# pliang279/factorized

Measured on AMD Instinct MI355X. Metric: training samples/sec (MOSI-shape, T=20, 3 modalities), higher is better.
Workload: dtype fp32; 1 GPU; MFM_KL_EF mosi canonical sizes, per-GPU B=32, T=20, D=325, train mode (fwd + joint loss + bwd + Adam), fp32 HIP; global_batch=32, seq_len=20, parallelism=dp1, params=477294, handover_failures=0, role_workgroups=True

## Files before the change

### factorized_amd/_lib.py

```python
import ctypes as C
import os

_HERE = os.path.dirname(os.path.abspath(__file__))
LIB_PATH = os.environ.get("MFM_LIB_PATH") or os.path.join(_HERE, "libmfm_hip.so")

MFM_KLEF_NPARAM = 78
MFM_LOSS_SLOTS = 8
MFM_MAX_SEQ = 6
ABI_VERSION = 5


class MfmError(RuntimeError):
    pass


class GemmDesc(C.Structure):
    _fields_ = [("a", C.c_void_p), ("b", C.c_void_p), ("c", C.c_void_p), ("c2", C.c_void_p),
                ("bias", C.c_void_p), ("bias2", C.c_void_p),
                ("a_sz", C.c_int64), ("a_sm", C.c_int64), ("a_sk", C.c_int64),
                ("b_sz", C.c_int64), ("b_sk", C.c_int64), ("b_sn", C.c_int64),
                ("c_sz", C.c_int64), ("ldc", C.c_int64), ("bias_sz", C.c_int64),
                ("m", C.c_int32), ("n", C.c_int32), ("k", C.c_int32), ("n_valid", C.c_int32),
                ("batch", C.c_int32), ("split_k", C.c_int32), ("accumulate", C.c_int32),
                ("alpha", C.c_float), ("a_bf16", C.c_int32), ("c_bf16", C.c_int32), ("reserved_", C.c_int32 * 2)]


class SeqDesc(C.Structure):
    _fields_ = [("gates", C.c_void_p), ("hs", C.c_void_p), ("cs", C.c_void_p),
                ("w_hh", C.c_void_p), ("w_ih", C.c_void_p), ("b_ih", C.c_void_p), ("b_hh", C.c_void_p),
                ("h_init", C.c_void_p), ("ld_init", C.c_int64),
                ("dh_ext", C.c_void_p), ("ld_dh", C.c_int64),
                ("d_h_init", C.c_void_p), ("ld_dinit", C.c_int64),
                ("h", C.c_int32), ("is_dec", C.c_int32), ("dc_ext", C.c_void_p), ("w_pack", C.c_void_p),
                ("store_bf16", C.c_int32), ("bf16_dot", C.c_int32), ("h_last", C.c_void_p)]


class MemDesc(C.Structure):
    _fields_ = [("a1", C.c_void_p), ("a2", C.c_void_p), ("chat", C.c_void_p),
                ("w1m", C.c_void_p), ("w2m", C.c_void_p), ("w1b", C.c_void_p), ("b1b", C.c_void_p),
                ("w2b", C.c_void_p), ("b2b", C.c_void_p),
                ("gam1", C.c_void_p), ("gam2", C.c_void_p), ("mems", C.c_void_p), ("mem_out", C.c_void_p),
                ("dmem_out", C.c_void_p), ("du1", C.c_void_p), ("du2", C.c_void_p), ("dchat", C.c_void_p),
                ("T", C.c_int32), ("B", C.c_int32), ("M", C.c_int32), ("H1", C.c_int32), ("H2", C.c_int32),
                ("train", C.c_int32), ("p1", C.c_float), ("p2", C.c_float), ("seed", C.c_uint64),
                ("seed_dev", C.c_void_p), ("ld_wm", C.c_int64), ("dchat_pre_tanh", C.c_int32), ("reserved_", C.c_int32)]


class AdamSpan(C.Structure):
    _fields_ = [("begin", C.c_int64), ("end", C.c_int64), ("step", C.c_int32), ("reserved", C.c_int32)]


MFM_ADAM_MAX_SPANS = 8


class SgdSpan(C.Structure):
    _fields_ = [("begin", C.c_int64), ("end", C.c_int64), ("lr", C.c_float), ("weight_decay", C.c_float),
                ("momentum", C.c_float), ("dampening", C.c_float), ("flags", C.c_int32), ("reserved", C.c_int32)]


MFM_SGD_MAX_SPANS = 112
MFM_SGD_NESTEROV, MFM_SGD_MAXIMIZE, MFM_SGD_FIRST = 1, 2, 4


class AdamExtSpan(C.Structure):
    _fields_ = [("begin", C.c_int64), ("end", C.c_int64), ("step", C.c_int32), ("flags", C.c_int32), ("lr", C.c_float),
                ("beta1", C.c_float), ("beta2", C.c_float), ("eps", C.c_float), ("weight_decay", C.c_float),
                ("reserved", C.c_int32)]


MFM_ADAMX_MAX_SPANS = 88
MFM_ADAMX_MAXIMIZE, MFM_ADAMX_AMSGRAD, MFM_ADAMX_DECOUPLED = 1, 2, 4


class ClipSpan(C.Structure):
    _fields_ = [("begin", C.c_int64), ("end", C.c_int64)]


MFM_CLIP_MAX_SPANS = 112
MFM_NORM_L2, MFM_NORM_INF, MFM_NORM_L1 = 0, 1, 2
MFM_AVG_SWA, MFM_AVG_EMA = 0, 1
MFM_KEEP_MIN, MFM_KEEP_MAX = 0, 1
MFM_KEEP_STATE_WORDS = 8
MFM_PLATEAU_MAX_GROUPS = 16
MFM_PLATEAU_MIN, MFM_PLATEAU_MAX = 0, 1
MFM_PLATEAU_REL, MFM_PLATEAU_ABS = 0, 1
MFM_PLATEAU_STATE_WORDS = 8


class PlateauGroups(C.Structure):
    _fields_ = [("lr", C.c_void_p * MFM_PLATEAU_MAX_GROUPS), ("min_lr", C.c_double * MFM_PLATEAU_MAX_GROUPS)]


class LossWeights(C.Structure):
    _fields_ = [("disc", C.c_float), ("gen_l", C.c_float), ("gen_a", C.c_float), ("gen_v", C.c_float), ("reg", C.c_float),
                ("write_disc_loss", C.c_int32)]


class PlanConfig(C.Structure):
    _fields_ = [("d_l", C.c_int32), ("d_a", C.c_int32), ("d_v", C.c_int32),
                ("zl", C.c_int32), ("za", C.c_int32), ("zv", C.c_int32), ("zy", C.c_int32),
                ("fl", C.c_int32), ("fa", C.c_int32), ("fv", C.c_int32), ("fy", C.c_int32),
                ("output_dim", C.c_int32), ("loss_kind", C.c_int32),
                ("T", C.c_int32), ("B", C.c_int32),
                ("lda_xl", C.c_float), ("lda_xa", C.c_float), ("lda_xv", C.c_float), ("lda_reg", C.c_float),
                ("drop_zy", C.c_float), ("drop_zl", C.c_float), ("drop_za", C.c_float),
                ("drop_zv", C.c_float), ("drop_y", C.c_float),
                ("reg_scale", C.c_float), ("precision", C.c_int32),
                ("variant", C.c_int32), ("hl", C.c_int32), ("ha", C.c_int32), ("hv", C.c_int32), ("mem_dim", C.c_int32),
                ("nn1", C.c_int32), ("nn2", C.c_int32), ("g1", C.c_int32), ("g2", C.c_int32),
                ("drop_nn1", C.c_float), ("drop_nn2", C.c_float), ("drop_g1", C.c_float), ("drop_g2", C.c_float)]


_SIGS = {
    "mfm_abi_version": (C.c_int, []),
    "mfm_last_error": (C.c_char_p, []),
    "mfm_device_cus": (C.c_int, []),
    "mfm_gemm_grouped_f32": (C.c_int, [C.POINTER(GemmDesc), C.c_int, C.c_void_p]),
    "mfm_gemm_grouped_bf16": (C.c_int, [C.POINTER(GemmDesc), C.c_int, C.c_void_p]),
    "mfm_lstm_pack_bytes": (C.c_int64, [C.c_int32, C.c_int32]),
    "mfm_lstm_pack_bf16": (C.c_int, [C.POINTER(SeqDesc), C.c_int, C.c_void_p]),
    "mfm_lstm_seq_fwd_bf16": (C.c_int, [C.POINTER(SeqDesc), C.c_int, C.c_int, C.c_int, C.c_void_p]),
    "mfm_lstm_seq_bwd_bf16": (C.c_int, [C.POINTER(SeqDesc), C.c_int, C.c_int, C.c_int, C.c_void_p]),
    "mfm_lstm_seq_fwd": (C.c_int, [C.POINTER(SeqDesc), C.c_int, C.c_int, C.c_int, C.c_void_p]),
    "mfm_lstm_seq_bwd": (C.c_int, [C.POINTER(SeqDesc), C.c_int, C.c_int, C.c_int, C.c_void_p]),
    "mfm_dw_bf16_lstm": (C.c_int, [C.c_void_p, C.c_int32, C.c_int32, C.c_void_p, C.c_int32, C.c_int32, C.c_void_p, C.c_int32,
                                   C.c_void_p, C.c_void_p, C.c_void_p, C.c_void_p, C.c_void_p, C.c_void_p]),
    "mfm_dw_f32_lstm": (C.c_int, [C.c_void_p, C.c_int32, C.c_int32, C.c_void_p, C.c_int32, C.c_int32, C.c_int32, C.c_void_p, C.c_int32,
                                  C.c_void_p, C.c_void_p, C.c_void_p, C.c_void_p, C.c_void_p, C.c_void_p]),
    "mfm_mmd_fwd_bwd": (C.c_int, [C.c_void_p, C.c_void_p, C.c_int32, C.c_int32, C.c_void_p, C.c_void_p, C.c_void_p]),
    "mfm_mfn_mem_fwd": (C.c_int, [C.POINTER(MemDesc), C.c_void_p]),
    "mfm_mfn_mem_bwd": (C.c_int, [C.POINTER(MemDesc), C.c_void_p]),
    "mfm_mse_fwd_bwd": (C.c_int, [C.c_void_p, C.c_void_p, C.c_int64, C.c_int64, C.c_int32, C.c_float,
                                  C.c_float, C.c_void_p, C.c_void_p, C.c_void_p]),
    "mfm_adam_flat": (C.c_int, [C.c_void_p, C.c_void_p, C.c_void_p, C.c_void_p, C.c_int64, C.c_int32,
                                C.c_float, C.c_float, C.c_float, C.c_float, C.c_float, C.c_void_p]),
    "mfm_adam_flat_spans": (C.c_int, [C.c_void_p, C.c_void_p, C.c_void_p, C.c_void_p, C.POINTER(AdamSpan), C.c_int32,
                                      C.c_float, C.c_float, C.c_float, C.c_float, C.c_float, C.c_void_p]),
    "mfm_adam_flat_guarded": (C.c_int, [C.c_void_p, C.c_void_p, C.c_void_p, C.c_void_p, C.c_int64, C.c_int32,
                                        C.c_float, C.c_float, C.c_float, C.c_float, C.c_float, C.c_void_p, C.c_void_p]),
    "mfm_adam_flat_dev": (C.c_int, [C.c_void_p, C.c_void_p, C.c_void_p, C.c_void_p, C.c_int64, C.c_void_p, C.c_void_p,
                                    C.c_float, C.c_float, C.c_float, C.c_float, C.c_void_p, C.c_void_p]),
    "mfm_adam_flat_spans_guarded": (C.c_int, [C.c_void_p, C.c_void_p, C.c_void_p, C.c_void_p, C.POINTER(AdamSpan), C.c_int32,
                                              C.c_float, C.c_float, C.c_float, C.c_float, C.c_float, C.c_void_p, C.c_void_p]),
    "mfm_sgd_flat_spans": (C.c_int, [C.c_void_p, C.c_void_p, C.c_void_p, C.POINTER(SgdSpan), C.c_int32, C.c_float, C.c_void_p]),
    "mfm_sgd_flat_spans_guarded": (C.c_int, [C.c_void_p, C.c_void_p, C.c_void_p, C.POINTER(SgdSpan), C.c_int32, C.c_float,
                                             C.c_void_p, C.c_void_p]),
    "mfm_adam_ext_flat_spans": (C.c_int, [C.c_void_p, C.c_void_p, C.c_void_p, C.c_void_p, C.c_void_p, C.POINTER(AdamExtSpan),
                                          C.c_int32, C.c_float, C.c_void_p]),
    "mfm_adam_ext_flat_spans_guarded": (C.c_int, [C.c_void_p, C.c_void_p, C.c_void_p, C.c_void_p, C.c_void_p,
                                                  C.POINTER(AdamExtSpan), C.c_int32, C.c_float, C.c_void_p, C.c_void_p]),
    "mfm_clip_workspace_floats": (C.c_int64, []),
    "mfm_clip_grad_norm_flat_spans": (C.c_int, [C.c_void_p, C.POINTER(ClipSpan), C.c_int32, C.c_int32, C.c_float, C.c_void_p,
                                                C.c_void_p, C.c_void_p, C.c_void_p]),
    "mfm_clip_grad_value_flat_spans": (C.c_int, [C.c_void_p, C.POINTER(ClipSpan), C.c_int32, C.c_float, C.c_void_p, C.c_void_p]),
    "mfm_avg_flat": (C.c_int, [C.c_void_p, C.c_void_p, C.c_int64, C.c_int64, C.c_int32, C.c_float, C.c_void_p, C.c_void_p,
                               C.c_void_p]),
    "mfm_keep_best_flat": (C.c_int, [C.c_void_p, C.c_void_p, C.c_int64, C.c_int64, C.c_int32, C.c_void_p, C.c_float, C.c_void_p,
                                     C.c_void_p]),
    "mfm_plateau_step": (C.c_int, [C.c_void_p, C.c_void_p, C.c_double, C.POINTER(PlateauGroups), C.c_int32, C.c_int32, C.c_int32,
                                   C.c_double, C.c_double, C.c_double, C.c_int32, C.c_int32, C.c_int32, C.c_void_p]),
    "mfm_dataset_gather": (C.c_int, [C.c_void_p, C.c_void_p, C.c_void_p, C.c_void_p, C.c_void_p, C.c_int64, C.c_int32, C.c_int32,
                                     C.c_int32, C.c_int32, C.c_int64, C.c_void_p]),
    "mfm_p2p_create": (C.c_int, [C.c_int32, C.c_int32, C.c_int64, C.POINTER(C.c_void_p)]),
    "mfm_p2p_handle_bytes": (C.c_int, []),
    "mfm_p2p_export": (C.c_int, [C.c_void_p, C.c_void_p]),
    "mfm_p2p_connect": (C.c_int, [C.c_void_p, C.c_void_p]),
    "mfm_p2p_local_base": (C.c_void_p, [C.c_void_p]),
    "mfm_p2p_connect_bases": (C.c_int, [C.c_void_p, C.POINTER(C.c_void_p)]),
    "mfm_p2p_allreduce": (C.c_int, [C.c_void_p, C.c_void_p, C.c_int64, C.c_void_p]),
    "mfm_p2p_allreduce_adam": (C.c_int, [C.c_void_p, C.c_void_p, C.c_void_p, C.c_void_p, C.c_void_p, C.c_int64,
                                         C.c_int32, C.c_float, C.c_float, C.c_float, C.c_float, C.c_float,
                                         C.c_void_p]),
    "mfm_p2p_allreduce_adam_guarded": (C.c_int, [C.c_void_p, C.c_void_p, C.c_void_p, C.c_void_p, C.c_void_p, C.c_int64,
                                                 C.c_int32, C.c_float, C.c_float, C.c_float, C.c_float, C.c_float,
                                                 C.c_int64, C.c_void_p]),
    "mfm_p2p_status": (C.c_int, [C.c_void_p, C.POINTER(C.c_int32)]),
    "mfm_p2p_wait_stats": (C.c_int, [C.c_void_p, C.POINTER(C.c_int64), C.c_int32]),
    "mfm_p2p_destroy": (None, [C.c_void_p]),
    "mfm_plan_num_params": (C.c_int, [C.c_int32]),
    "mfm_plan_set_gauss": (C.c_int, [C.c_void_p, C.c_void_p]),
    "mfm_plan_create": (C.c_int, [C.POINTER(PlanConfig), C.POINTER(C.c_int64), C.c_int64,
                                  C.POINTER(C.c_void_p)]),
    "mfm_plan_destroy": (None, [C.c_void_p]),
    "mfm_plan_workspace_bytes": (C.c_int64, [C.c_void_p]),
    "mfm_plan_init_workspace": (C.c_int, [C.c_void_p, C.c_void_p, C.c_void_p]),
    "mfm_plan_forward": (C.c_int, [C.c_void_p, C.c_void_p, C.c_void_p, C.c_void_p, C.c_int, C.c_uint64,
                                   C.c_void_p, C.c_void_p, C.c_void_p, C.c_void_p, C.c_void_p,
                                   C.c_void_p, C.c_void_p]),
    "mfm_plan_backward": (C.c_int, [C.c_void_p, C.c_void_p, C.c_void_p, C.c_void_p, C.c_int, C.c_void_p,
                                    C.c_void_p, C.c_void_p]),
    "mfm_plan_backward_ext": (C.c_int, [C.c_void_p] * 11),
    "mfm_plan_forward_train": (C.c_int, [C.c_void_p, C.c_void_p, C.c_void_p, C.c_uint64, C.c_void_p, C.c_void_p, C.c_void_p]),
    "mfm_plan_backward_weighted": (C.c_int, [C.c_void_p, C.c_void_p, C.c_void_p, C.c_void_p, C.POINTER(LossWeights),
                                             C.c_void_p, C.c_void_p, C.c_void_p]),
    "mfm_plan_out_layout": (C.c_int, [C.c_void_p, C.POINTER(C.c_int64)]),
    "mfm_plan_host_status": (C.c_int, [C.c_void_p, C.POINTER(C.POINTER(C.c_uint32))]),
    "mfm_plan_grad_step": (C.c_int, [C.c_void_p, C.c_void_p, C.c_void_p, C.c_void_p, C.c_void_p, C.c_uint64,
                                     C.c_void_p, C.c_void_p, C.c_void_p]),
    "mfm_plan_train_step": (C.c_int, [C.c_void_p, C.c_void_p, C.c_void_p, C.c_void_p, C.c_void_p,
                                      C.c_void_p, C.c_void_p, C.c_uint64, C.c_int32, C.c_float,
                                      C.c_float, C.c_void_p, C.c_void_p, C.c_void_p]),
    "mfm_plan_train_step_staged": (C.c_int, [C.c_void_p, C.c_void_p, C.c_void_p, C.c_void_p, C.c_void_p,
                                             C.c_void_p, C.c_void_p, C.c_uint64, C.c_int32, C.POINTER(AdamSpan),
                                             C.c_int32, C.c_float, C.c_float, C.c_void_p, C.c_void_p, C.c_void_p]),
    "mfm_plan_set_option": (C.c_int, [C.c_void_p, C.c_char_p, C.c_int64]),
    "mfm_plan_set_option_str": (C.c_int, [C.c_void_p, C.c_char_p, C.c_char_p]),
    "mfm_plan_get_option": (C.c_int, [C.c_void_p, C.c_char_p, C.POINTER(C.c_int64)]),
    "mfm_plan_state_layout": (C.c_int, [C.c_void_p, C.POINTER(C.c_int64)]),
    "mfm_plan_clear_status": (C.c_int, [C.c_void_p, C.c_void_p, C.c_void_p]),
    "mfm_plan_latent_layout": (C.c_int, [C.c_void_p, C.POINTER(C.c_int64)]),
    "mfm_plan_seq_layout": (C.c_int, [C.c_void_p, C.c_int32, C.POINTER(C.c_int64)]),
    "mfm_plan_mfn_layout": (C.c_int, [C.c_void_p, C.POINTER(C.c_int64)]),
    "mfm_plan_flops_per_step": (C.c_double, [C.c_void_p]),
    "mfm_plan_bytes_per_step": (C.c_double, [C.c_void_p]),
    "mfm_plan_set_timing": (C.c_int, [C.c_void_p, C.c_int]),
    "mfm_plan_set_timing_every": (C.c_int, [C.c_void_p, C.c_int]),
    "mfm_plan_num_kernels": (C.c_int, []),
    "mfm_plan_kernel_name": (C.c_char_p, [C.c_int]),
    "mfm_plan_collect_timing": (C.c_int, [C.c_void_p, C.POINTER(C.c_double), C.POINTER(C.c_int64)]),
    "mfm_timing_bracket_overhead_ms": (C.c_int, [C.c_void_p, C.POINTER(C.c_double)]),
    "mfm_plan_kernel_flops": (C.c_double, [C.c_void_p, C.c_int]),
}

_lib = None


def lib():
    global _lib
    if _lib is None:
        if not os.path.exists(LIB_PATH):
            raise MfmError(
                "factorized_amd: %s is missing. Build the gfx950 HIP library first:\n"
                "    python -c 'import __graft_entry__ as g; g.build()'   (or factorized_amd/csrc/build.sh)\n"
                "There is no CPU fallback for this package." % LIB_PATH)
        import torch
        L = C.CDLL(LIB_PATH)
        for name, (res, args) in _SIGS.items():
            fn = getattr(L, name)
            fn.restype = res
            fn.argtypes = args
        if L.mfm_abi_version() != ABI_VERSION:
            raise MfmError("libmfm_hip.so ABI version %d, binding expects %d" % (L.mfm_abi_version(), ABI_VERSION))
        _lib = L
    return _lib


def check(rc, what=""):
    if rc != 0:
        msg = lib().mfm_last_error()
        raise MfmError("%s failed (%d): %s" % (what or "libmfm_hip call", rc,
                                               msg.decode() if msg else "?"))


def exported_names():
    return list(_SIGS)
```

### factorized_amd/csrc/dec_fc1.hip

```cpp
#include <hip/hip_runtime.h>
#include "internal.h"
#include "lstamp.h"

namespace mfm {

constexpr int FC1_THREADS = 512;
constexpr int FC1_WAVES = 8;
constexpr int FC1_ROWS = 16;
constexpr int FC1_MAXF = 8;
constexpr int FC1_KS2W = 4;
constexpr int FC1_LD = 16 * FC1_MAXF + 4;
constexpr int FC1_OOB = 0x7FFFFFF0;

__device__ __forceinline__ float rnd_bf16(float x, bool on) { return on ? (float)(__bf16)x : x; }

__global__ __launch_bounds__(FC1_THREADS) void dec_fc1_kernel(const DecFc1Launch L) {
  __shared__ __attribute__((aligned(16))) float Ht[FC1_ROWS * FC1_LD];
  __shared__ __attribute__((aligned(16))) float Dx[FC1_ROWS * FC1_LD];
  __shared__ __attribute__((aligned(16))) float Pt[(FC1_WAVES / 2) * FC1_ROWS * FC1_LD];
  __shared__ float red[FC1_WAVES];
  LSTAMP(2, 0);
  int m = 0;
#pragma unroll
  for (int i = 1; i < 3; ++i)
    if (i < L.n_items && (int)blockIdx.x >= L.it[i].tile_begin) m = i;
  const DecFc1Item& I = L.it[m];
  const int d = I.d, h = I.h, Hp = I.Hp;
  const int local = (int)blockIdx.x - I.tile_begin;
  const int cg = local % I.col_groups;
  const int row0 = (local / I.col_groups) * FC1_ROWS;
  const int NF1 = (d + 15) >> 4;
  const int f0 = cg * I.frags_per_group, nfw = min(I.frags_per_group, NF1 - f0);
  const int tid = threadIdx.x, lane = tid & 63, wave = tid >> 6;
  const int bi = lane & 15, q = lane >> 4;
  const int J = Hp >> 4;

  const int per_row = Hp >> 2;
  const int hr = tid / per_row, hk = (tid - hr * per_row) << 2;
  f32x4 hreg = f32x4{0.f, 0.f, 0.f, 0.f};
  if (hr < FC1_ROWS && row0 + hr < L.rows) hreg = *reinterpret_cast<const f32x4*>(I.hs + (int64_t)(row0 + hr) * Hp + hk);
  const __amdgpu_buffer_rsrc_t wres = __builtin_amdgcn_make_buffer_rsrc((void*)I.w, 0, d * h * 4, 0x00020000);
  const int n = (f0 + wave) * 16 + bi;
  const bool cok = (int)(wave < nfw) & (int)(n < d);
  f32x4 w1[FC1_MAXF];
#pragma unroll
  for (int j = 0; j < FC1_MAXF; ++j) {
    const bool ok = (int)cok & (int)(j < J);
    w1[j] = __builtin_bit_cast(f32x4, __builtin_amdgcn_raw_buffer_load_b128(wres, ok ? (n * h + 16 * j + 4 * q) * 4 : FC1_OOB, 0, 0));
  }
  const int KS = nfw * 4;
  const int per = (KS + FC1_WAVES - 1) / FC1_WAVES;
  const int ks0 = wave * per;
  float w2[FC1_KS2W][FC1_MAXF];
#pragma unroll
  for (int i = 0; i < FC1_KS2W; ++i) {
    const int k = f0 * 16 + 4 * (ks0 + i) + q;
#pragma unroll
    for (int f = 0; f < FC1_MAXF; ++f) {
      const int c = f * 16 + bi;
      const bool ok = (int)(L.with_bwd != 0) & (int)(i < per) & (int)(ks0 + i < KS) & (int)(k < d) & (int)(c < h);
      w2[i][f] = __builtin_bit_cast(float, __builtin_amdgcn_raw_buffer_load_b32(wres, ok ? (k * h + c) * 4 : FC1_OOB, 0, 0));
    }
  }
  float xv[4];
#pragma unroll
  for (int r = 0; r < 4; ++r) {
    const int row = row0 + 4 * q + r;
    xv[r] = (cok && row < L.rows) ? I.x[(int64_t)row * I.ldx + n] : 0.0f;
  }
  const float bv = cok ? I.bias[n] : 0.0f;
  const bool rb = L.bf16 != 0;
  if (rb) {
#pragma unroll
    for (int e = 0; e < 4; ++e) hreg[e] = rnd_bf16(hreg[e], true);
  }
  if (hr < FC1_ROWS) *reinterpret_cast<f32x4*>(Ht + hr * FC1_LD + hk) = hreg;
  lds_barrier();
  LSTAMP(2, 1);

  f32x4 acc1 = f32x4{0.f, 0.f, 0.f, 0.f};
  if (wave < nfw) {
#pragma unroll
    for (int j = 0; j < FC1_MAXF; ++j) {
      const f32x4 hv = *reinterpret_cast<const f32x4*>(Ht + bi * FC1_LD + 16 * min(j, J - 1) + 4 * q);
#pragma unroll
      for (int e = 0; e < 4; ++e) acc1 = mma16x16x4(hv[e], rnd_bf16(w1[j][e], rb), acc1);
    }
  }
  float lsum = 0.0f;
  if (wave < nfw) {
#pragma unroll
    for (int r = 0; r < 4; ++r) {
      const int row = 4 * q + r;
      float dx = 0.0f;
      if (cok && row0 + row < L.rows) {
        const float xh = acc1[r] + bv;
        const float diff = xh - xv[r];
        lsum = fmaf(diff, diff, lsum);
        dx = I.grad_scale * diff;
        const int64_t o = (int64_t)(row0 + row) * d + n;
        if (I.xhat) I.xhat[o] = xh;
        if (I.dxhat) I.dxhat[o] = dx;
      }
      Dx[row * FC1_LD + wave * 16 + bi] = rnd_bf16(dx, rb);
    }
  }
#pragma unroll
  for (int o = 32; o >= 1; o >>= 1) lsum += __shfl_xor(lsum, o, 64);
  if (lane == 0) red[wave] = lsum;
  lds_barrier();
  if (tid == 0 && I.loss) {
    float s = 0.0f;
#pragma unroll
    for (int w = 0; w < FC1_WAVES; ++w) s += red[w];
    atomicAdd(I.loss, s * I.inv_count);
  }
  LSTAMP(2, 2);
  if (!L.with_bwd) return;

  {
    f32x4 acc2[FC1_MAXF];
#pragma unroll
    for (int f = 0; f < FC1_MAXF; ++f) acc2[f] = f32x4{0.f, 0.f, 0.f, 0.f};
#pragma unroll
    for (int i = 0; i < FC1_KS2W; ++i) {
      const float a = Dx[bi * FC1_LD + 4 * min(ks0 + i, KS - 1) + q];
#pragma unroll
      for (int f = 0; f < FC1_MAXF; ++f) acc2[f] = mma16x16x4(a, rnd_bf16(w2[i][f], rb), acc2[f]);
    }
    float* P = Pt + (wave & 3) * FC1_ROWS * FC1_LD;
    if (wave >= 4) {
#pragma unroll
      for (int f = 0; f < FC1_MAXF; ++f)
#pragma unroll
        for (int r = 0; r < 4; ++r) P[(4 * q + r) * FC1_LD + f * 16 + bi] = acc2[f][r];
    }
    lds_barrier();
    if (wave < 4) {
#pragma unroll
      for (int f = 0; f < FC1_MAXF; ++f)
#pragma unroll
        for (int r = 0; r < 4; ++r) P[(4 * q + r) * FC1_LD + f * 16 + bi] += acc2[f][r];
    }
  }
  lds_barrier();
  if (hr < FC1_ROWS && row0 + hr < L.rows) {
    f32x4 s = *reinterpret_cast<const f32x4*>(Pt + hr * FC1_LD + hk);
#pragma unroll
    for (int w = 1; w < FC1_WAVES / 2; ++w) s += *reinterpret_cast<const f32x4*>(Pt + (w * FC1_ROWS + hr) * FC1_LD + hk);
    float* o = I.dhs + (int64_t)(row0 + hr) * Hp + hk;
    if (I.col_groups == 1) {
      *reinterpret_cast<f32x4*>(o) = s;
    } else {
#pragma unroll
      for (int e = 0; e < 4; ++e) atomicAdd(o + e, s[e]);
    }
  }
  LSTAMP_W(2, 15);
}

int dec_fc1_launch(DecFc1Launch& L, bool dhs_zeroed, hipStream_t stream) {
  MFM_REQUIRE(L.n_items >= 1 && L.n_items <= 3 && L.rows >= 1, "dec fc1: bad launch");
  int tiles = 0;
  const int row_tiles = (L.rows + FC1_ROWS - 1) / FC1_ROWS;
  for (int i = 0; i < L.n_items; ++i) {
    DecFc1Item& I = L.it[i];
    MFM_REQUIRE(I.hs && I.w && I.bias && I.x && I.d >= 1 && I.h >= 1 && I.Hp >= I.h && (I.Hp & 15) == 0, "dec fc1: item %d", i);
    MFM_REQUIRE(!L.with_bwd || I.dhs, "dec fc1: item %d: backward without a dH buffer", i);
    if (I.Hp > 16 * FC1_MAXF || (int64_t)I.d * I.h >= ((int64_t)1 << 28)) return MFM_ERR_UNSUPPORTED;
    const int NF1 = (I.d + 15) >> 4;
    if (NF1 > FC1_MAXF && !(dhs_zeroed || !L.with_bwd)) return MFM_ERR_UNSUPPORTED;
    I.frags_per_group = std::min(FC1_MAXF, NF1);
    I.col_groups = (NF1 + I.frags_per_group - 1) / I.frags_per_group;
    I.tile_begin = tiles;
    tiles += row_tiles * I.col_groups;
  }
  LSTAMP_BIND();
  MFM_LAUNCH_TIMED(dec_fc1_kernel, dim3(tiles), dim3(FC1_THREADS), 0, stream, L);
  MFM_LAUNCH_CHECK("dec_fc1_kernel");
  return MFM_OK;
}

}
```

### factorized_amd/csrc/lstamp.h

```cpp
#pragma once
#ifndef MFM_LAUNCH_STAMP
#define MFM_LAUNCH_STAMP 0
#endif

#if MFM_LAUNCH_STAMP
#include <hip/hip_runtime.h>

namespace mfm {
constexpr int LST_KERNELS = 6;
constexpr int LST_BLOCKS = 512;
constexpr int LST_POINTS = 32;
namespace {
__device__ unsigned long long* g_lstamp;
}
unsigned long long* lstamp_buffer();
static inline void lstamp_bind() {
  static bool done = false;
  if (done) return;
  unsigned long long* p = lstamp_buffer();
  (void)hipMemcpyToSymbol(HIP_SYMBOL(g_lstamp), &p, sizeof(p));
  done = true;
}
__device__ __forceinline__ void lstamp(int kid, int point, bool wait_loads = false) {
  if (threadIdx.x < 64) {
    if (wait_loads) asm volatile("s_waitcnt vmcnt(0) lgkmcnt(0)" ::: "memory");
    if (threadIdx.x == 0 && blockIdx.x < LST_BLOCKS && point < LST_POINTS)
      g_lstamp[((long)kid * LST_BLOCKS + blockIdx.x) * LST_POINTS + point] = wall_clock64();
  }
}
}
#define LSTAMP(kid, pt) ::mfm::lstamp(kid, pt)
#define LSTAMP_W(kid, pt) ::mfm::lstamp(kid, pt, true)
#define LSTAMP_BIND() ::mfm::lstamp_bind()
#else
#define LSTAMP(kid, pt) ((void)0)
#define LSTAMP_W(kid, pt) ((void)0)
#define LSTAMP_BIND() ((void)0)
#endif
```

### include/mfm_hip.h

```cpp
#ifndef MFM_HIP_H_
#define MFM_HIP_H_

#include <stddef.h>
#include <stdint.h>

#ifdef __cplusplus
extern "C" {
#endif

#define MFM_OK 0
#define MFM_ERR_ARG (-1)
#define MFM_ERR_HIP (-2)
#define MFM_ERR_UNSUPPORTED (-3)

#define MFM_ABI_VERSION 5

int mfm_abi_version(void);
const char* mfm_last_error(void);
int mfm_device_cus(void);

typedef struct MfmGemmDesc {
  const float* a; const float* b; float* c; float* c2;
  const float* bias; const float* bias2;
  int64_t a_sz, a_sm, a_sk;
  int64_t b_sz, b_sk, b_sn;
  int64_t c_sz, ldc, bias_sz;
  int32_t m, n, k, n_valid, batch, split_k, accumulate;
  float alpha;
  int32_t a_bf16, c_bf16;
  int32_t reserved_[2];
} MfmGemmDesc;

int mfm_gemm_grouped_f32(const MfmGemmDesc* descs , int count, void* stream);
int mfm_gemm_grouped_bf16(const MfmGemmDesc* descs , int count, void* stream);

#define MFM_MAX_SEQ 6
typedef struct MfmSeqDesc {
  float* gates; float* hs; float* cs;
  const float* w_hh; const float* w_ih; const float* b_ih; const float* b_hh;
  const float* h_init; int64_t ld_init;
  const float* dh_ext;
  int64_t ld_dh;
  float* d_h_init;
  int64_t ld_dinit;
  int32_t h, is_dec;
  const float* dc_ext;
  void* w_pack;
  int32_t store_bf16;
  int32_t bf16_dot;
  float* h_last;
} MfmSeqDesc;

int mfm_lstm_seq_fwd(const MfmSeqDesc* descs , int count, int T, int B, void* stream);

int64_t mfm_lstm_pack_bytes(int32_t h, int32_t is_dec);
int mfm_lstm_pack_bf16(const MfmSeqDesc* descs , int count, void* stream);
int mfm_lstm_seq_fwd_bf16(const MfmSeqDesc* descs , int count, int T, int B, void* stream);
int mfm_lstm_seq_bwd_bf16(const MfmSeqDesc* descs , int count, int T, int B, void* stream);

int mfm_lstm_seq_bwd(const MfmSeqDesc* descs , int count, int T, int B, void* stream);

int mfm_dw_bf16_lstm(const void* dA, int32_t rows, int32_t h, const void* xb, int32_t ldx, int32_t dx, const void* hs,
                     int32_t shift, float* dw_ih, float* dw_hh, float* dw_hh2, float* db_ih, float* db_hh, void* stream);
int mfm_dw_f32_lstm(const float* dA, int32_t rows, int32_t h, const float* x, int32_t ldx, int32_t xcol0, int32_t dx,
                    const float* hs, int32_t shift, float* dw_ih, float* dw_hh, float* dw_hh2, float* db_ih, float* db_hh,
                    void* stream);

int mfm_mse_fwd_bwd(const float* xhat, const float* x, int64_t ldx, int64_t rows, int32_t d,
                    float inv_count, float grad_scale, float* dxhat, float* loss_slot, void* stream);

typedef struct MfmMemDesc {
  float* a1; float* a2;
  const float* chat;
  const float* w1m; const float* w2m;
  const float* w1b; const float* b1b;
  const float* w2b; const float* b2b;
  float* gam1; float* gam2; float* mems;
  float* mem_out;
  const float* dmem_out;
  float* du1; float* du2; float* dchat;
  int32_t T, B, M, H1, H2, train;
  float p1, p2;
  uint64_t seed;
  const uint64_t* seed_dev;
  int64_t ld_wm;
  int32_t dchat_pre_tanh;
  int32_t reserved_;
} MfmMemDesc;

int mfm_mfn_mem_fwd(const MfmMemDesc* desc , void* stream);
int mfm_mfn_mem_bwd(const MfmMemDesc* desc , void* stream);

int mfm_mmd_fwd_bwd(const float* z, const float* gauss, int32_t B, int32_t dim, float* loss ,
                    float* dz , void* stream);

int mfm_adam_flat(float* p, const float* g, float* m, float* v, int64_t n, int32_t step, float lr,
                  float beta1, float beta2, float eps, float grad_scale, void* stream);

int mfm_adam_flat_guarded(float* p, const float* g, float* m, float* v, int64_t n, int32_t step, float lr,
                          float beta1, float beta2, float eps, float grad_scale, const float* guard, void* stream);

int mfm_adam_flat_dev(float* p, const float* g, float* m, float* v, int64_t n, int32_t* step_dev, const float* lr_dev,
                      float beta1, float beta2, float eps, float grad_scale, const float* guard, void* stream);

#define MFM_ADAM_MAX_SPANS 8
typedef struct MfmAdamSpan { int64_t begin, end; int32_t step; int32_t reserved; } MfmAdamSpan;
int mfm_adam_flat_spans(float* p, const float* g, float* m, float* v, const MfmAdamSpan* spans , int32_t nspans,
                        float lr, float beta1, float beta2, float eps, float grad_scale, void* stream);
int mfm_adam_flat_spans_guarded(float* p, const float* g, float* m, float* v, const MfmAdamSpan* spans , int32_t nspans,
                                float lr, float beta1, float beta2, float eps, float grad_scale, const float* guard, void* stream);

#define MFM_SGD_MAX_SPANS 112
#define MFM_SGD_NESTEROV 1
#define MFM_SGD_MAXIMIZE 2
#define MFM_SGD_FIRST 4
typedef struct MfmSgdSpan {
  int64_t begin, end;
  float lr, weight_decay, momentum, dampening;
  int32_t flags;
  int32_t reserved;
} MfmSgdSpan;
int mfm_sgd_flat_spans(float* p, const float* g, float* buf, const MfmSgdSpan* spans , int32_t nspans, float grad_scale,
                       void* stream);
int mfm_sgd_flat_spans_guarded(float* p, const float* g, float* buf, const MfmSgdSpan* spans , int32_t nspans,
                               float grad_scale, const float* guard, void* stream);

#define MFM_ADAMX_MAX_SPANS 88
#define MFM_ADAMX_MAXIMIZE 1
#define MFM_ADAMX_AMSGRAD 2
#define MFM_ADAMX_DECOUPLED 4
typedef struct MfmAdamExtSpan {
  int64_t begin, end;
  int32_t step;
  int32_t flags;
  float lr, beta1, beta2, eps, weight_decay;
  int32_t reserved;
} MfmAdamExtSpan;
int mfm_adam_ext_flat_spans(float* p, const float* g, float* m, float* v, float* vmax, const MfmAdamExtSpan* spans ,
                            int32_t nspans, float grad_scale, void* stream);
int mfm_adam_ext_flat_spans_guarded(float* p, const float* g, float* m, float* v, float* vmax,
                                    const MfmAdamExtSpan* spans , int32_t nspans, float grad_scale, const float* guard,
                                    void* stream);

#define MFM_CLIP_MAX_SPANS 112
#define MFM_NORM_L2 0
#define MFM_NORM_INF 1
#define MFM_NORM_L1 2
typedef struct MfmClipSpan {
  int64_t begin, end;
} MfmClipSpan;
int64_t mfm_clip_workspace_floats(void);
int mfm_clip_grad_norm_flat_spans(float* g, const MfmClipSpan* spans , int32_t nspans, int32_t norm_kind, float max_norm,
                                  float* ws, float* total_norm , const float* guard, void* stream);
int mfm_clip_grad_value_flat_spans(float* g, const MfmClipSpan* spans , int32_t nspans, float clip_value,
                                   const float* guard, void* stream);

#define MFM_AVG_SWA 0
#define MFM_AVG_EMA 1
int mfm_avg_flat(float* avg, const float* p, int64_t begin, int64_t end, int32_t kind, float w, int64_t* n_averaged ,
                 int32_t* ticket , void* stream);

#define MFM_KEEP_MIN 0
#define MFM_KEEP_MAX 1
typedef struct MfmKeepBestState {
  float best_value;
  int32_t calls;
  int32_t best_call;
  int32_t taken;
  int32_t ticket;
  int32_t reserved_[3];
} MfmKeepBestState;
int mfm_keep_best_flat(float* best, const float* p, int64_t begin, int64_t end, int32_t mode, const float* metric_dev ,
                       float metric, MfmKeepBestState* state , void* stream);

#define MFM_PLATEAU_MAX_GROUPS 16
#define MFM_PLATEAU_MIN 0
#define MFM_PLATEAU_MAX 1
#define MFM_PLATEAU_REL 0
#define MFM_PLATEAU_ABS 1
typedef struct MfmPlateauState {
  double best;
  int32_t num_bad_epochs;
  int32_t cooldown_counter;
  int32_t last_epoch;
  int32_t reduced;
  int32_t reductions;
  int32_t reserved_;
} MfmPlateauState;
typedef struct MfmPlateauGroups {
  float* lr[MFM_PLATEAU_MAX_GROUPS];
  double min_lr[MFM_PLATEAU_MAX_GROUPS];
} MfmPlateauGroups;
int mfm_plateau_step(MfmPlateauState* state , const float* metric_dev , double metric,
                     const MfmPlateauGroups* groups , int32_t n_groups, int32_t mode, int32_t threshold_mode, double factor,
                     double threshold, double eps, int32_t patience, int32_t cooldown, int32_t epoch ,
                     void* stream);

int mfm_dataset_gather(float* X, void* y, const float* X_pool, const void* y_pool, const int64_t* perm , int64_t N,
                       int32_t nb, int32_t T, int32_t B, int32_t D, int64_t ybytes, void* stream);

int mfm_p2p_create(int32_t nranks , int32_t rank, int64_t max_elems, void** handle);
int mfm_p2p_handle_bytes(void);
int mfm_p2p_export(void* handle, void* out );
int mfm_p2p_connect(void* handle, const void* all_handles );
void* mfm_p2p_local_base(void* handle);
int mfm_p2p_connect_bases(void* handle, const void* const* bases );
int mfm_p2p_allreduce(void* handle, float* buf , int64_t n , void* stream);
int mfm_p2p_allreduce_adam(void* handle, float* grads, float* p, float* m, float* v, int64_t n, int32_t step,
                           float lr, float beta1, float beta2, float eps, float grad_scale, void* stream);
int mfm_p2p_allreduce_adam_guarded(void* handle, float* grads, float* p, float* m, float* v, int64_t n, int32_t step,
                                   float lr, float beta1, float beta2, float eps, float grad_scale, int64_t guard_index,
                                   void* stream);
int mfm_p2p_status(void* handle, int32_t* timed_out );
int mfm_p2p_wait_stats(void* handle, int64_t* out , int32_t reset);
void mfm_p2p_destroy(void* handle);

#define MFM_KLEF_NPARAM 78
#define MFM_LOSS_SLOTS 8

typedef struct MfmPlanConfig {
  int32_t d_l, d_a, d_v;
  int32_t zl, za, zv, zy;
  int32_t fl, fa, fv, fy;
  int32_t output_dim;
  int32_t loss_kind;
  int32_t T, B;
  float lda_xl, lda_xa, lda_xv, lda_reg;
  float drop_zy, drop_zl, drop_za, drop_zv, drop_y;
  float reg_scale;
  int32_t precision;
  int32_t variant;
  int32_t hl, ha, hv;
  int32_t mem_dim;
  int32_t nn1, nn2, g1, g2;
  float drop_nn1, drop_nn2, drop_g1, drop_g2;
} MfmPlanConfig;

typedef struct MfmPlan MfmPlan;

int mfm_plan_num_params(int32_t variant);
int mfm_plan_create(const MfmPlanConfig* cfg, const int64_t* param_offsets ,
                    int64_t n_params_total, MfmPlan** out);
int mfm_plan_set_gauss(MfmPlan* plan, const float* gauss);
void mfm_plan_destroy(MfmPlan* plan);
int64_t mfm_plan_workspace_bytes(const MfmPlan* plan);

int mfm_plan_init_workspace(MfmPlan* plan, void* workspace, void* stream);

int mfm_plan_forward(MfmPlan* plan, const float* params, const float* x, const void* y, int train,
                     uint64_t seed, void* workspace, float* xhat_l, float* xhat_a, float* xhat_v,
                     float* y_hat, float* losses, void* stream);

int mfm_plan_backward(MfmPlan* plan, const float* params, const float* x, const void* y, int stage,
                      void* workspace, float* grads, void* stream);

int mfm_plan_backward_ext(MfmPlan* plan, const float* params, const float* x, const float* d_xhat_l,
                          const float* d_xhat_a, const float* d_xhat_v, const float* d_yhat,
                          const float* d_reg, void* workspace, float* grads, void* stream);

typedef struct MfmLossWeights { float disc, gen_l, gen_a, gen_v, reg; int32_t write_disc_loss; } MfmLossWeights;
int mfm_plan_forward_train(MfmPlan* plan, const float* params, const float* x, uint64_t seed, void* workspace,
                           float* grads_to_zero, void* stream);
int mfm_plan_backward_weighted(MfmPlan* plan, const float* params, const float* x, const void* y,
                               const MfmLossWeights* w , void* workspace, float* grads, void* stream);
int mfm_plan_out_layout(const MfmPlan* plan, int64_t* out );

int mfm_plan_grad_step(MfmPlan* plan, const float* params, float* grads, const float* x, const void* y,
                       uint64_t seed, void* workspace, float* losses, void* stream);

int mfm_plan_train_step(MfmPlan* plan, float* params, float* grads, float* adam_m, float* adam_v,
                        const float* x, const void* y, uint64_t seed, int32_t step, float lr,
                        float grad_scale, void* workspace, float* losses, void* stream);

int mfm_plan_train_step_staged(MfmPlan* plan, float* params, float* grads, float* adam_m, float* adam_v,
                               const float* x, const void* y, uint64_t seed, int32_t stage,
                               const MfmAdamSpan* spans , int32_t nspans, float lr, float grad_scale,
                               void* workspace, float* losses, void* stream);

int mfm_plan_set_option(MfmPlan* plan, const char* key, int64_t value);
int mfm_plan_set_option_str(MfmPlan* plan, const char* key, const char* value);
int mfm_plan_get_option(const MfmPlan* plan, const char* key, int64_t* value);

int mfm_plan_state_layout(const MfmPlan* plan, int64_t* out );
int mfm_plan_host_status(MfmPlan* plan, uint32_t** out );
int mfm_plan_clear_status(MfmPlan* plan, void* workspace, void* stream);

int mfm_plan_latent_layout(const MfmPlan* plan, int64_t* out );

int mfm_plan_mfn_layout(const MfmPlan* plan, int64_t* out );

int mfm_plan_seq_layout(const MfmPlan* plan, int32_t which, int64_t* out );

double mfm_plan_flops_per_step(const MfmPlan* plan);
double mfm_plan_bytes_per_step(const MfmPlan* plan);

int mfm_plan_set_timing(MfmPlan* plan, int mask);
int mfm_plan_set_timing_every(MfmPlan* plan, int every);
int mfm_plan_num_kernels(void);
const char* mfm_plan_kernel_name(int kid);
int mfm_plan_collect_timing(MfmPlan* plan, double* sum_ms, int64_t* count);
int mfm_timing_bracket_overhead_ms(void* stream, double* ms_out);
double mfm_plan_kernel_flops(const MfmPlan* plan, int kid);

#ifdef __cplusplus
}
#endif
#endif
```

Measured before the change: 225,000 samples/s.

## Reuse fc1 weight fragments via LDS transpose for backward dgrad in decoder kernel

The decoder fc1 kernel no longer issues a second set of scalar global loads for the backward weight tile. Instead it writes the already-loaded forward weight fragments into a dynamic LDS buffer, transposed, and each wave computes one output column block of dhs directly, which removes the cross-wave partial-sum reduction and its extra barriers. The forward accumulation is split into four independent accumulators to shorten the MFMA dependency chain, and the xhat/dxhat stores are deferred until after the backward MMA. It also adds a C entry point and a Python binding for the kernel, plus timing stamp hooks. In exchange it needs more dynamic LDS per block, which may reduce occupancy.

```diff
diff --git a/factorized_amd/_lib.py b/factorized_amd/_lib.py
--- a/factorized_amd/_lib.py
+++ b/factorized_amd/_lib.py
@@ -74,6 +74,13 @@
 
 class ClipSpan(C.Structure):
     _fields_ = [("begin", C.c_int64), ("end", C.c_int64)]
+
+
+class DecFc1Item(C.Structure):
+    _fields_ = [("hs", C.c_void_p), ("w", C.c_void_p), ("bias", C.c_void_p), ("x", C.c_void_p),
+                ("xhat", C.c_void_p), ("dxhat", C.c_void_p), ("dhs", C.c_void_p), ("loss", C.c_void_p),
+                ("ldx", C.c_int64), ("d", C.c_int32), ("h", C.c_int32), ("Hp", C.c_int32),
+                ("inv_count", C.c_float), ("grad_scale", C.c_float), ("pad_", C.c_int32)]
 
 
 MFM_CLIP_MAX_SPANS = 112
@@ -153,6 +160,7 @@
     "mfm_clip_grad_norm_flat_spans": (C.c_int, [C.c_void_p, C.POINTER(ClipSpan), C.c_int32, C.c_int32, C.c_float, C.c_void_p,
                                                 C.c_void_p, C.c_void_p, C.c_void_p]),
     "mfm_clip_grad_value_flat_spans": (C.c_int, [C.c_void_p, C.POINTER(ClipSpan), C.c_int32, C.c_float, C.c_void_p, C.c_void_p]),
+    "mfm_dec_fc1_f32": (C.c_int, [C.POINTER(DecFc1Item), C.c_int32, C.c_int32, C.c_int32, C.c_int32, C.c_int32, C.c_void_p]),
     "mfm_avg_flat": (C.c_int, [C.c_void_p, C.c_void_p, C.c_int64, C.c_int64, C.c_int32, C.c_float, C.c_void_p, C.c_void_p,
                                C.c_void_p]),
     "mfm_keep_best_flat": (C.c_int, [C.c_void_p, C.c_void_p, C.c_int64, C.c_int64, C.c_int32, C.c_void_p, C.c_float, C.c_void_p,
diff --git a/factorized_amd/csrc/dec_fc1.hip b/factorized_amd/csrc/dec_fc1.hip
--- a/factorized_amd/csrc/dec_fc1.hip
+++ b/factorized_amd/csrc/dec_fc1.hip
@@ -1,4 +1,5 @@
 #include <hip/hip_runtime.h>
+#include <atomic>
 #include "internal.h"
 #include "lstamp.h"
 
@@ -8,7 +9,6 @@
 constexpr int FC1_WAVES = 8;
 constexpr int FC1_ROWS = 16;
 constexpr int FC1_MAXF = 8;
-constexpr int FC1_KS2W = 4;
 constexpr int FC1_LD = 16 * FC1_MAXF + 4;
 constexpr int FC1_OOB = 0x7FFFFFF0;
 
@@ -17,8 +17,8 @@
 __global__ __launch_bounds__(FC1_THREADS) void dec_fc1_kernel(const DecFc1Launch L) {
   __shared__ __attribute__((aligned(16))) float Ht[FC1_ROWS * FC1_LD];
   __shared__ __attribute__((aligned(16))) float Dx[FC1_ROWS * FC1_LD];
-  __shared__ __attribute__((aligned(16))) float Pt[(FC1_WAVES / 2) * FC1_ROWS * FC1_LD];
   __shared__ float red[FC1_WAVES];
+  extern __shared__ __attribute__((aligned(16))) float Wt[];
   LSTAMP(2, 0);
   int m = 0;
 #pragma unroll
@@ -34,6 +34,7 @@
   const int tid = threadIdx.x, lane = tid & 63, wave = tid >> 6;
   const int bi = lane & 15, q = lane >> 4;
   const int J = Hp >> 4;
+  const bool bwd = L.with_bwd != 0;
 
   const int per_row = Hp >> 2;
   const int hr = tid / per_row, hk = (tid - hr * per_row) << 2;
@@ -48,20 +49,6 @@
     const bool ok = (int)cok & (int)(j < J);
     w1[j] = __builtin_bit_cast(f32x4, __builtin_amdgcn_raw_buffer_load_b128(wres, ok ? (n * h + 16 * j + 4 * q) * 4 : FC1_OOB, 0, 0));
   }
-  const int KS = nfw * 4;
-  const int per = (KS + FC1_WAVES - 1) / FC1_WAVES;
-  const int ks0 = wave * per;
-  float w2[FC1_KS2W][FC1_MAXF];
-#pragma unroll
-  for (int i = 0; i < FC1_KS2W; ++i) {
-    const int k = f0 * 16 + 4 * (ks0 + i) + q;
-#pragma unroll
-    for (int f = 0; f < FC1_MAXF; ++f) {
-      const int c = f * 16 + bi;
-      const bool ok = (int)(L.with_bwd != 0) & (int)(i < per) & (int)(ks0 + i < KS) & (int)(k < d) & (int)(c < h);
-      w2[i][f] = __builtin_bit_cast(float, __builtin_amdgcn_raw_buffer_load_b32(wres, ok ? (k * h + c) * 4 : FC1_OOB, 0, 0));
-    }
-  }
   float xv[4];
 #pragma unroll
   for (int r = 0; r < 4; ++r) {
@@ -77,85 +64,104 @@
   if (hr < FC1_ROWS) *reinterpret_cast<f32x4*>(Ht + hr * FC1_LD + hk) = hreg;
   lds_barrier();
   LSTAMP(2, 1);
-
-  f32x4 acc1 = f32x4{0.f, 0.f, 0.f, 0.f};
-  if (wave < nfw) {
-#pragma unroll
-    for (int j = 0; j < FC1_MAXF; ++j) {
-      const f32x4 hv = *reinterpret_cast<const f32x4*>(Ht + bi * FC1_LD + 16 * min(j, J - 1) + 4 * q);
-#pragma unroll
-      for (int e = 0; e < 4; ++e) acc1 = mma16x16x4(hv[e], rnd_bf16(w1[j][e], rb), acc1);
-    }
-  }
+  LSTAMP_V(2, 10, 5);
+
+  f32x4 acc1[4];
+#pragma unroll
+  for (int e = 0; e < 4; ++e) acc1[e] = f32x4{0.f, 0.f, 0.f, 0.f};
+  float xh[4] = {0.f, 0.f, 0.f, 0.f}, dxr[4] = {0.f, 0.f, 0.f, 0.f};
   float lsum = 0.0f;
   if (wave < nfw) {
 #pragma unroll
+    for (int j = 0; j < FC1_MAXF; ++j) {
+      if (j < J) {
+        const f32x4 hv = *reinterpret_cast<const f32x4*>(Ht + bi * FC1_LD + 16 * j + 4 * q);
+        f32x4 wv;
+#pragma unroll
+        for (int e = 0; e < 4; ++e) wv[e] = rnd_bf16(w1[j][e], rb);
+#pragma unroll
+        for (int e = 0; e < 4; ++e) acc1[e] = mma16x16x4(hv[e], wv[e], acc1[e]);
+        if (bwd) {
+#pragma unroll
+          for (int e = 0; e < 4; ++e) {
+            const int u = 16 * j + 4 * q + e;
+            Wt[u * FC1_LD + wave * 16 + bi] = u < h ? wv[e] : 0.0f;
+          }
+        }
+      }
+    }
+    LSTAMP_W(2, 11);
+    const f32x4 s1 = (acc1[0] + acc1[1]) + (acc1[2] + acc1[3]);
+#pragma unroll
     for (int r = 0; r < 4; ++r) {
       const int row = 4 * q + r;
-      float dx = 0.0f;
+      xh[r] = s1[r] + bv;
+      dxr[r] = 0.0f;
       if (cok && row0 + row < L.rows) {
-        const float xh = acc1[r] + bv;
-        const float diff = xh - xv[r];
+        const float diff = xh[r] - xv[r];
         lsum = fmaf(diff, diff, lsum);
-        dx = I.grad_scale * diff;
-        const int64_t o = (int64_t)(row0 + row) * d + n;
-        if (I.xhat) I.xhat[o] = xh;
-        if (I.dxhat) I.dxhat[o] = dx;
-      }
-      Dx[row * FC1_LD + wave * 16 + bi] = rnd_bf16(dx, rb);
+        dxr[r] = I.grad_scale * diff;
+      }
+      Dx[row * FC1_LD + wave * 16 + bi] = rnd_bf16(dxr[r], rb);
     }
   }
 #pragma unroll
   for (int o = 32; o >= 1; o >>= 1) lsum += __shfl_xor(lsum, o, 64);
   if (lane == 0) red[wave] = lsum;
+  LSTAMP(2, 12);
   lds_barrier();
-  if (tid == 0 && I.loss) {
+  LSTAMP(2, 2);
+
+  f32x4 acc2[4];
+#pragma unroll
+  for (int e = 0; e < 4; ++e) acc2[e] = f32x4{0.f, 0.f, 0.f, 0.f};
+  const bool w2on = (int)bwd & (int)(wave < J);
+  if (w2on) {
+    f32x4 av[FC1_MAXF], wv[FC1_MAXF];
+#pragma unroll
+    for (int j = 0; j < FC1_MAXF; ++j) {
+      if (j < nfw) {
+        av[j] = *reinterpret_cast<const f32x4*>(Dx + bi * FC1_LD + 16 * j + 4 * q);
+        wv[j] = *reinterpret_cast<const f32x4*>(Wt + (wave * 16 + bi) * FC1_LD + 16 * j + 4 * q);
+      }
+    }
+#pragma unroll
+    for (int j = 0; j < FC1_MAXF; ++j) {
+      if (j < nfw) {
+#pragma unroll
+        for (int e = 0; e < 4; ++e) acc2[e] = mma16x16x4(av[j][e], wv[j][e], acc2[e]);
+      }
+    }
+  }
+  if (cok) {
+#pragma unroll
+    for (int r = 0; r < 4; ++r) {
+      const int row = row0 + 4 * q + r;
+      if (row < L.rows) {
+        const int64_t o = (int64_t)row * d + n;
+        if (I.xhat) I.xhat[o] = xh[r];
+        if (I.dxhat) I.dxhat[o] = dxr[r];
+      }
+    }
+  }
+  if (tid == FC1_THREADS - 64 && I.loss) {
     float s = 0.0f;
 #pragma unroll
     for (int w = 0; w < FC1_WAVES; ++w) s += red[w];
     atomicAdd(I.loss, s * I.inv_count);
   }
-  LSTAMP(2, 2);
-  if (!L.with_bwd) return;
-
-  {
-    f32x4 acc2[FC1_MAXF];
-#pragma unroll
-    for (int f = 0; f < FC1_MAXF; ++f) acc2[f] = f32x4{0.f, 0.f, 0.f, 0.f};
-#pragma unroll
-    for (int i = 0; i < FC1_KS2W; ++i) {
-      const float a = Dx[bi * FC1_LD + 4 * min(ks0 + i, KS - 1) + q];
-#pragma unroll
-      for (int f = 0; f < FC1_MAXF; ++f) acc2[f] = mma16x16x4(a, rnd_bf16(w2[i][f], rb), acc2[f]);
-    }
-    float* P = Pt + (wave & 3) * FC1_ROWS * FC1_LD;
-    if (wave >= 4) {
-#pragma unroll
-      for (int f = 0; f < FC1_MAXF; ++f)
-#pragma unroll
-        for (int r = 0; r < 4; ++r) P[(4 * q + r) * FC1_LD + f * 16 + bi] = acc2[f][r];
-    }
-    lds_barrier();
-    if (wave < 4) {
-#pragma unroll
-      for (int f = 0; f < FC1_MAXF; ++f)
-#pragma unroll
-        for (int r = 0; r < 4; ++r) P[(4 * q + r) * FC1_LD + f * 16 + bi] += acc2[f][r];
-    }
-  }
-  lds_barrier();
-  if (hr < FC1_ROWS && row0 + hr < L.rows) {
-    f32x4 s = *reinterpret_cast<const f32x4*>(Pt + hr * FC1_LD + hk);
-#pragma unroll
-    for (int w = 1; w < FC1_WAVES / 2; ++w) s += *reinterpret_cast<const f32x4*>(Pt + (w * FC1_ROWS + hr) * FC1_LD + hk);
-    float* o = I.dhs + (int64_t)(row0 + hr) * Hp + hk;
-    if (I.col_groups == 1) {
-      *reinterpret_cast<f32x4*>(o) = s;
-    } else {
-#pragma unroll
-      for (int e = 0; e < 4; ++e) atomicAdd(o + e, s[e]);
-    }
-  }
+  if (w2on) {
+    const f32x4 s2 = (acc2[0] + acc2[1]) + (acc2[2] + acc2[3]);
+    float* o = I.dhs + (int64_t)(row0 + 4 * q) * Hp + wave * 16 + bi;
+#pragma unroll
+    for (int r = 0; r < 4; ++r) {
+      if (row0 + 4 * q + r < L.rows) {
+        if (I.col_groups == 1) o[r * Hp] = s2[r];
+        else atomicAdd(o + r * Hp, s2[r]);
+      }
+    }
+  }
+  LSTAMP(2, 13);
   LSTAMP_W(2, 15);
 }
 
@@ -175,10 +181,37 @@
     I.tile_begin = tiles;
     tiles += row_tiles * I.col_groups;
   }
+  int max_hp = 0;
+  for (int i = 0; i < L.n_items; ++i) max_hp = std::max(max_hp, L.it[i].Hp);
+  const size_t smem = L.with_bwd ? (size_t)max_hp * FC1_LD * sizeof(float) : 0;
+  static std::atomic<unsigned long long> lds_attr_set{0};
+  int dev = 0;
+  MFM_HIP_CHECK(hipGetDevice(&dev));
+  const unsigned long long dev_bit = 1ull << (dev & 63);
+  if (!(lds_attr_set.load(std::memory_order_acquire) & dev_bit)) {
+    MFM_HIP_CHECK(hipFuncSetAttribute((const void*)dec_fc1_kernel, hipFuncAttributeMaxDynamicSharedMemorySize, 16 * FC1_MAXF * FC1_LD * (int)sizeof(float)));
+    lds_attr_set.fetch_or(dev_bit, std::memory_order_release);
+  }
   LSTAMP_BIND();
-  MFM_LAUNCH_TIMED(dec_fc1_kernel, dim3(tiles), dim3(FC1_THREADS), 0, stream, L);
+  MFM_LAUNCH_TIMED(dec_fc1_kernel, dim3(tiles), dim3(FC1_THREADS), smem, stream, L);
   MFM_LAUNCH_CHECK("dec_fc1_kernel");
   return MFM_OK;
 }
 
 }
+
+extern "C" int mfm_dec_fc1_f32(const MfmDecFc1Item* items, int32_t count, int32_t rows, int32_t with_bwd, int32_t bf16_operands,
+                               int32_t dhs_zeroed, void* stream) {
+  MFM_REQUIRE(items && count >= 1 && count <= 3, "dec fc1: 1..3 items");
+  mfm::DecFc1Launch L;
+  memset(&L, 0, sizeof(L));
+  L.n_items = count; L.rows = rows; L.with_bwd = with_bwd ? 1 : 0; L.bf16 = bf16_operands ? 1 : 0;
+  for (int i = 0; i < count; ++i) {
+    mfm::DecFc1Item& I = L.it[i];
+    const MfmDecFc1Item& s = items[i];
+    I.hs = s.hs; I.w = s.w; I.bias = s.bias; I.x = s.x; I.ldx = s.ldx;
+    I.xhat = s.xhat; I.dxhat = s.dxhat; I.dhs = s.dhs; I.loss = s.loss;
+    I.d = s.d; I.h = s.h; I.Hp = s.Hp; I.inv_count = s.inv_count; I.grad_scale = s.grad_scale;
+  }
+  return mfm::dec_fc1_launch(L, dhs_zeroed != 0, (hipStream_t)stream);
+}
diff --git a/factorized_amd/csrc/lstamp.h b/factorized_amd/csrc/lstamp.h
--- a/factorized_amd/csrc/lstamp.h
+++ b/factorized_amd/csrc/lstamp.h
@@ -28,12 +28,19 @@
       g_lstamp[((long)kid * LST_BLOCKS + blockIdx.x) * LST_POINTS + point] = wall_clock64();
   }
 }
+template <int N>
+__device__ __forceinline__ void lstamp_v(int kid, int point) {
+  if (threadIdx.x < 64) asm volatile("s_waitcnt vmcnt(%0)" ::"n"(N) : "memory");
+  lstamp(kid, point);
+}
 }
 #define LSTAMP(kid, pt) ::mfm::lstamp(kid, pt)
+#define LSTAMP_V(kid, pt, n) ::mfm::lstamp_v<n>(kid, pt)
 #define LSTAMP_W(kid, pt) ::mfm::lstamp(kid, pt, true)
 #define LSTAMP_BIND() ::mfm::lstamp_bind()
 #else
 #define LSTAMP(kid, pt) ((void)0)
 #define LSTAMP_W(kid, pt) ((void)0)
+#define LSTAMP_V(kid, pt, n) ((void)0)
 #define LSTAMP_BIND() ((void)0)
 #endif
diff --git a/include/mfm_hip.h b/include/mfm_hip.h
--- a/include/mfm_hip.h
+++ b/include/mfm_hip.h
@@ -154,6 +154,17 @@
                                   float* ws, float* total_norm , const float* guard, void* stream);
 int mfm_clip_grad_value_flat_spans(float* g, const MfmClipSpan* spans , int32_t nspans, float clip_value,
                                    const float* guard, void* stream);
+
+typedef struct MfmDecFc1Item {
+  const float* hs; const float* w; const float* bias; const float* x;
+  float* xhat; float* dxhat; float* dhs; float* loss;
+  int64_t ldx;
+  int32_t d, h, Hp;
+  float inv_count, grad_scale;
+  int32_t pad_;
+} MfmDecFc1Item;
+int mfm_dec_fc1_f32(const MfmDecFc1Item* items , int32_t count, int32_t rows, int32_t with_bwd, int32_t bf16_operands,
+                    int32_t dhs_zeroed, void* stream);
 
 #define MFM_AVG_SWA 0
 #define MFM_AVG_EMA 1
```

After: 228,100 samples/s, median of 6. 1.4% higher.
